# JihyongOh/DeMFI

Hardware: AMD Instinct MI355X
Metric: interpolated frames/sec @720p x8 MFI (N_tst=3) (higher is better)
Workload: dtype f16; 1 GPU; DeMFI-Net_rb N_tst=3, x8 MFI, 720x1280 (padded 736x1280), fp16, clip-parallel windows, random-init weights; uint8 frames host->HBM->host inside the timed region (PNG codec excluded), 8 distinct windows; graph=True, parallelism=clip1, n_ctx=7, n_trunk=3

## Files before the change

demfi_amd/_lib.py:

```python
import ctypes as C
import os

_HERE = os.path.dirname(os.path.abspath(__file__))
LIB_PATH = os.environ.get('DEMFI_HIP_LIB') or os.path.join(_HERE, 'csrc', 'libdemfi_hip.so')

F16, F32 = 0, 1
ABI_VERSION = 8
ACT_NONE, ACT_RELU, ACT_TANH, ACT_SIGMOID = 0, 1, 2, 3
MODE_STORE, MODE_MUL, MODE_GRU = 0, 1, 2
BT601, BT709 = 0, 1
SITING_420JPEG, SITING_420MPEG2 = 0, 1
YUV_LAYOUT = {'420': 0, '422': 1, '444': 2, 'mono': 3}
OWNERS = ('sep', 'wstream7', 'ws2', 'wstream3', 'c64', 'narrow_nhwc', 'narrow_thin', 'general')
OWNERS_COUT_PERM = frozenset(range(6))
MAX_PIECES, MAX_CHUNKS, MAX_SEGS, MAX_OCTS = 48, 40, 8, 32


class View(C.Structure):
    _fields_ = [('ptr', C.c_void_p), ('sx', C.c_int64), ('sy', C.c_int64), ('sc', C.c_int64), ('sb', C.c_int64),
                ('is_f32', C.c_int32), ('_pad', C.c_int32)]


class Piece(C.Structure):
    _fields_ = [('v', View), ('nch', C.c_int32), ('lds_ch', C.c_int32), ('up_shift', C.c_int32), ('fat', C.c_int32)]
# ... 176 lines not shown
                                   C.POINTER(C.c_int64)]),
    'demfi_png_info': (C.c_int, [C.c_void_p, C.c_int64, C.POINTER(C.c_int), C.POINTER(C.c_int)]),
    'demfi_png_decode': (C.c_int, [C.c_void_p, C.c_int64, C.c_void_p, C.c_int64, C.c_int, C.c_int]),
    'demfi_conv_build': (C.c_int, [C.c_int, C.c_int, C.c_int, C.c_int, C.c_int, C.c_void_p, C.c_void_p, C.c_int, C.c_int,
                                   C.c_int, C.c_int, C.POINTER(ConvSrc), C.c_int, C.POINTER(ConvDst), C.c_int, C.POINTER(Conv),
                                   C.c_void_p, C.POINTER(C.c_int64), C.c_void_p, C.POINTER(C.c_int32)]),
    'demfi_ctx_create': (C.c_int, [C.c_int, C.c_int, C.c_int, C.c_int, C.POINTER(HParams), C.c_int, C.c_int,
                                   C.POINTER(C.c_void_p)]),
    'demfi_ctx_destroy': (C.c_int, [C.c_void_p]),
    'demfi_gru_sep_create': (C.c_int, [C.c_int, C.c_int, C.c_int, C.c_int, C.POINTER(C.c_void_p)]),
    'demfi_fgac_create': (C.c_int, [C.c_int, C.c_int, C.c_int, C.c_int, C.POINTER(C.c_void_p)]),
    'demfi_operator_run': (C.c_int, [C.c_void_p, C.c_void_p]),
    'demfi_load_weight': (C.c_int, [C.c_void_p, C.c_char_p, C.c_void_p, C.POINTER(C.c_int64), C.c_int]),
    'demfi_ctx_workspace_bytes': (C.c_int64, [C.c_void_p]),
    'demfi_workspace_bytes': (C.c_int64, [C.c_int, C.c_int, C.c_int, C.c_int, C.c_int, C.c_int]),
    'demfi_ctx_bind': (C.c_int, [C.c_void_p, C.c_void_p, C.c_int64, C.c_int, C.c_void_p]),
    'demfi_ctx_weight_region': (C.c_int, [C.c_void_p, C.POINTER(C.c_int64), C.POINTER(C.c_int64)]),
    'demfi_ctx_buffer': (C.c_int, [C.c_void_p, C.c_int, C.c_int, C.c_char_p, C.POINTER(C.c_int64), C.POINTER(C.c_int32),
                                   C.POINTER(C.c_int32)]),
    'demfi_ingest_u8': (C.c_int, [C.c_void_p, C.c_int, C.c_void_p, C.c_int, C.c_int, C.c_void_p]),
    'demfi_ingest_u16': (C.c_int, [C.c_void_p, C.c_int, C.c_void_p, C.c_int, C.c_int, C.c_int, C.c_void_p]),
    'demfi_ingest_u16_rect': (C.c_int, [C.c_void_p, C.c_int, C.c_void_p, C.c_int, C.c_int, C.c_int, C.c_int, C.c_int, C.c_int, C.c_int,
                                        C.c_void_p]),
    'demfi_forward_trunk_body': (C.c_int, [C.c_void_p, C.c_int, C.c_void_p]),
    'demfi_forward_trunk': (C.c_int, [C.c_void_p, C.c_int, C.c_void_p, C.c_void_p]),
    'demfi_forward_t': (C.c_int, [C.c_void_p, C.c_int, C.c_int, C.c_int, C.c_void_p]),
    'demfi_forward_tb': (C.c_int, [C.c_void_p, C.c_int, C.c_int, C.c_void_p]),
    'demfi_forward_tb_final': (C.c_int, [C.c_void_p, C.c_int, C.c_int, C.c_void_p]),
    'demfi_ctx_num_ops': (C.c_int, [C.c_void_p, C.c_int, C.c_int, C.c_int, C.c_int]),
    'demfi_ctx_get_op': (C.c_int, [C.c_void_p, C.c_int, C.c_int, C.c_int, C.c_int, C.c_int, C.POINTER(Op)]),
    'demfi_ctx_num_convs': (C.c_int, [C.c_void_p]),
    'demfi_ctx_conv_desc': (C.POINTER(Conv), [C.c_void_p, C.c_int]),
    'demfi_conv_owner': (C.c_int, [C.POINTER(Conv)]),
    'demfi_run_op': (C.c_int, [C.c_void_p, C.POINTER(Op), C.c_void_p]),
    'demfi_graph_begin': (C.c_int, [C.c_void_p]),
    'demfi_graph_end': (C.c_int, [C.c_void_p, C.POINTER(C.c_void_p)]),
    'demfi_graph_launch': (C.c_int, [C.c_void_p, C.c_void_p]),
    'demfi_graph_destroy': (C.c_int, [C.c_void_p]),
}

EXPORTS = tuple(_SIGS)
_lib = None


class DemfiError(RuntimeError):
    pass


def load():
    global _lib
    if _lib is not None:
        return _lib
    if not os.path.exists(LIB_PATH):
        raise RuntimeError('demfi_amd: %s not found -- build it with demfi_amd/csrc/build.sh (or '
                           '__graft_entry__.build()); there is no CPU/PyTorch fallback for the forward path'
                           % LIB_PATH)
    lib = C.CDLL(LIB_PATH)
    for name, (res, args) in _SIGS.items():
        fn = getattr(lib, name)
        fn.restype = res
        fn.argtypes = args
    if lib.demfi_abi_version() != ABI_VERSION:
        raise RuntimeError('demfi_amd: ABI version mismatch')
    _lib = lib
    return lib

# ... 16 lines not shown
```

demfi_amd/csrc/conv.hip:

```cpp
#include "conv_common.h"

namespace {

static bool persist_out_eligible(const demfi_conv* h, bool allow_tanh = false);

bool persist_eligible(const demfi_conv* h)
{
    if (h->dtype != DEMFI_F16 || h->stride != 1 || h->kh != 3 || h->kw != 3 || h->pad_y != 1 || h->pad_x != 1) return false;
    if (h->n_chunks != 1 || h->n_pieces != 1 || h->chunks[0].nks != 4 || h->rec_bytes != 128) return false;
    const demfi_piece& p = h->pieces[0];
    if (!p.fat || p.nch != 64 || p.up_shift != 0 || !p.v.ptr || p.v.is_f32) return false;
    if (!persist_out_eligible(h, h->nco == 2)) return false;
    return demfi_c64_strides_ok(h);
}

static bool thin_out_eligible(const demfi_conv* h)
{
    if (h->nco != 1 || h->cout_pad != 32 || !h->zero_page || h->inH != h->H || h->inW != h->W || h->sub_seg[0] >= 0) return false;
    bool any = false;
    for (int g = 0; g < 4; ++g) {
        if (h->oct_n[g] == 0) continue;
        any = true;
        const demfi_seg& sg = h->segs[h->oct_seg[g]];
        if (sg.mode != DEMFI_MODE_STORE || sg.scale != 1 || sg.dy != 0 || sg.dx != 0) return false;
// ... 121 lines not shown
        if (!ok) return demfi_set_error(DEMFI_ERR_ARG, "demfi_conv2d: subtile %d is not eligible for the staged epilogue", sb);
    }
    hipStream_t st = (hipStream_t)stream;
    const int owner = demfi_conv_owner(h);
    if (h->pack.ptr != nullptr) {
        bool ok = owner == DEMFI_OWNER_NARROW_THIN && h->pack.sc == 1 && !h->pack.is_f32;
        for (int g = 0; g < 4; ++g) ok = ok && (h->pack_oct_ch[g] < 0 || (h->pack_oct_ch[g] % 4 == 0 && h->oct_n[g] > 0));
        if (!ok) return demfi_set_error(DEMFI_ERR_ARG, "demfi_conv2d: packed copy (demfi_conv.pack) on a layer that is not a thin-output fp16 narrow layer, or malformed");
    }
    if ((h->cout_perm != 0) != demfi_persist_eligible(h))
        return demfi_set_error(DEMFI_ERR_ARG, h->cout_perm ? "demfi_conv2d: descriptor packed for a persistent kernel (cout_perm) but not eligible for one (zero_page missing?)"
                                                           : "demfi_conv2d: persistent-kernel layer without cout_perm (build the descriptor with demfi_conv_build)");
    switch (owner) {
    case DEMFI_OWNER_SEP: return demfi_sep_launch(h, dev, st);
    case DEMFI_OWNER_WSTREAM7: return demfi_wstream_launch(h, dev, st);
    case DEMFI_OWNER_WS2: return demfi_ws2_launch(h, dev, st);
    case DEMFI_OWNER_WSTREAM3: return demfi_wstream3_launch(h, dev, st);
    case DEMFI_OWNER_C64: return demfi_c64_launch(h, dev, st);
    case DEMFI_OWNER_NARROW_NHWC: return demfi_narrow_launch(h, dev, st, false);
    case DEMFI_OWNER_NARROW_THIN: return demfi_narrow_launch(h, dev, st, true);
    default: return demfi_conv_general_launch(h, dev, st, (size_t)lds);
    }
}

#ifdef DEMFI_TRACE
extern "C" int demfi_trace_dump(unsigned long long* out, int64_t n)
{
    const int64_t have = TR_N;
    if (!out || n < have) return demfi_set_error(DEMFI_ERR_ARG, "demfi_trace_dump: need room for %lld entries", (long long)have);
    DEMFI_HIP_CHECK(hipDeviceSynchronize());
    for (int64_t i = 0; i < have; ++i) out[i] = 0;
    int st = demfi_c64_trace_collect(out);
    if (st >= 0) st = demfi_narrow_trace_collect(out);
    if (st >= 0) st = demfi_sep_trace_collect(out);
    if (st >= 0) st = demfi_wstream_trace_collect(out);
    return st < 0 ? st : (int)have;
}
#endif
```

demfi_amd/csrc/conv_kernels.h:

```cpp
#pragma once
#include <hip/hip_runtime.h>
#include "demfi_hip.h"

int demfi_conv_general_launch(const demfi_conv* h, const demfi_conv* dev, hipStream_t st, size_t lds);
int demfi_c64_launch(const demfi_conv* h, const demfi_conv* dev, hipStream_t st);
bool demfi_c64_strides_ok(const demfi_conv* h);
int demfi_narrow_launch(const demfi_conv* h, const demfi_conv* dev, hipStream_t st, bool thin);
bool demfi_sep_eligible(const demfi_conv* h);
int demfi_sep_launch(const demfi_conv* h, const demfi_conv* dev, hipStream_t st);
bool demfi_wstream_eligible(const demfi_conv* h, int ks = 7, int nch = 2);
int demfi_wstream_launch(const demfi_conv* h, const demfi_conv* dev, hipStream_t st);
int demfi_wstream3_launch(const demfi_conv* h, const demfi_conv* dev, hipStream_t st);
int demfi_c64_trace_collect(unsigned long long* acc);
int demfi_narrow_trace_collect(unsigned long long* acc);
int demfi_sep_trace_collect(unsigned long long* acc);
int demfi_wstream_trace_collect(unsigned long long* acc);
```

demfi_amd/csrc/conv_narrow.hip:

```cpp
#include "conv_common.h"

namespace {

template <int REC, int KS = 3> struct NarrowCfg {
    static constexpr int LW = TW + KS - 1, LH = TH + KS - 1, NP = LW * LH, PAD = KS / 2, NTAPS = KS * KS;
    static constexpr int NKS = REC / 32;
    static constexpr int SL = REC / 16;
    static constexpr int PPI = 1024 / REC;
    static constexpr int NI = (NP + PPI - 1) / PPI;
    static constexpr int TILE_BYTES = NI * 1024;
#ifndef DEMFI_N64_NBUF
#define DEMFI_N64_NBUF 3
#define DEMFI_N64_NDMA 4
#define DEMFI_N32_NDMA 2
#endif
    static constexpr int NBUF = REC == 128 ? 2 : (REC == 64 ? DEMFI_N64_NBUF : 4);
    static_assert(KS == 3 || (KS == 7 && REC == 32), "7x7: one 16-channel k-step per tap (49 KiB of resident weights)");
    static constexpr int NDMA = REC == 128 ? 4 : (REC == 64 ? DEMFI_N64_NDMA : (KS == 7 ? 2 : DEMFI_N32_NDMA));
    static_assert((NBUF - 1) * ((NI + NDMA - 1) / NDMA) <= 63, "a DMA wave's tiles in flight must be countable in vmcnt");
    static __device__ __forceinline__ int swz(int col) { return REC == 128 ? (col >> 1) & 7 : (REC == 64 ? (col >> 2) & 3 : (col >> 4) & 1); }
    static constexpr size_t lds_bytes(int nco) { return (size_t)NTAPS * NKS * nco * 1024 + (size_t)NBUF * TILE_BYTES + 1024; }
};

struct NarrowFrag { uint4 a[2], b0, b1; };

__device__ __forceinline__ void quad_transpose4(float (&a)[4], int lane)
{
    auto dpp = [](float v, auto CTRL) {
        return __builtin_bit_cast(float, __builtin_amdgcn_update_dpp(0, __builtin_bit_cast(int, v), decltype(CTRL)::value, 0xF, 0xF, false));
    };
    const bool b0 = lane & 1, b1 = lane & 2;
    float p[4], y[4], q[4];
#pragma unroll
    for (int j = 0; j < 4; ++j) p[j] = dpp(a[j], std::integral_constant<int, 0xB1>{});
    y[0] = b0 ? p[1] : a[0]; y[1] = b0 ? a[1] : p[0]; y[2] = b0 ? p[3] : a[2]; y[3] = b0 ? a[3] : p[2];
#pragma unroll
    for (int j = 0; j < 4; ++j) q[j] = dpp(y[j], std::integral_constant<int, 0x4E>{});
    a[0] = b1 ? q[2] : y[0]; a[1] = b1 ? q[3] : y[1]; a[2] = b1 ? y[2] : q[0]; a[3] = b1 ? y[3] : q[1];
}
#ifndef DEMFI_THIN_REGW_G128
#define DEMFI_THIN_REGW_G128 6
#endif
template <int NCO, int REC, int EPI, int KS = 3, int NDMA = NarrowCfg<REC, KS>::NDMA, int NOCT = 4, bool PACK = false, bool P7 = false>
__global__ __launch_bounds__(NT + 64 * NDMA, 1) void conv3x3_narrow_persist_kernel(const demfi_conv* __restrict__ d)
{
    static_assert(!P7 || (KS == 7 && NCO == 1 && REC == 32), "paired taps: the 7x7 / 16-channel / 32-cout instantiation");
    constexpr bool RES = EPI == 1, THIN = EPI == 2;
    constexpr bool REGW = THIN && KS == 3 && NCO == 1;
    constexpr int RG = (REGW && REC == 128 && NOCT == 1 && !PACK) ? DEMFI_THIN_REGW_G128 : 0;
    constexpr bool WLDS = RG < (REC / 32) * 3 || !REGW;
    static_assert(!PACK || THIN, "packed copy: thin epilogue only");
    static_assert(!THIN || NCO == 1, "thin epilogue: one 32-cout subtile");
    using Cfg = NarrowCfg<REC, KS>;
    constexpr int P_LW = Cfg::LW, P_NP = Cfg::NP, PAD = Cfg::PAD;
    constexpr int NKS = Cfg::NKS, SL = Cfg::SL, NI = Cfg::NI, NBUF = Cfg::NBUF, TILE_BYTES = Cfg::TILE_BYTES;
// ... 403 lines not shown
                    for (int p = 0; p < 2; ++p) quad_transpose4(vv[g][p], lane);
                }
#pragma unroll
                for (int g = 0; g < NOCT; ++g) {
#pragma unroll
                    for (int p = 0; p < 2; ++p) {
#pragma unroll
                        for (int j = 0; j < 4; ++j) vv[g][p][j] = vv[g][p][j] + tr[g][p][j];
                    }
                    apply_act_n<4>(vv[g][0], t_act[g]);
                    apply_act_n<4>(vv[g][1], t_act[g]);
                }
#pragma unroll
                for (int g = 0; g < NOCT; ++g) {
#pragma unroll
                    for (int p = 0; p < 2; ++p) {
                        const int oyv = oy0 + wave * 2 + p;
                        if (oyv < H && q4 < t_nq[g]) {
                            f4_t o;
#pragma unroll
                            for (int j = 0; j < 4; ++j) o[j] = vv[g][p][j];
                            *gp<f4_t>(t_dstq[g] + bimg * t_dsb[g] + (int64_t)oyv * t_dsy[g] + ox0 + (lx & ~3)) = o;
                        }
                    }
                }
                if constexpr (PACK) {
#pragma unroll
                    for (int g = 0; g < NOCT; ++g) {
                        if (pk_dst[g] == nullptr) continue;
#pragma unroll
                        for (int p = 0; p < 2; ++p) {
                            quad_transpose4(vv[g][p], lane);
                            const int oyv = oy0 + wave * 2 + p;
                            if (oyv < H) {
                                h4_t o;
#pragma unroll
                                for (int j = 0; j < 4; ++j) o[j] = j < t_nq[g] ? (half_t)vv[g][p][j] : (half_t)0.0f;
                                *gp<h4_t>(pk_dst[g] + bimg * pk_sb + (int64_t)oyv * pk_sy + (int64_t)(ox0 + lx) * pk_sx) = o;
                            }
                        }
                    }
                }
                TRACE_STAMP(wave, k, 3);
                continue;
            }
#pragma unroll
            for (int g = 0; g < NOCT; ++g) {
                if (t_on[g] == 0) continue;
                const f4_t bq = t_bias[g];
#pragma unroll
                for (int p = 0; p < 2; ++p) {
                    float v[4];
#pragma unroll
                    for (int j = 0; j < 4; ++j) v[j] = (acc[0][p][g * 4 + j] + bq[j]) + tr[g][p][j];
                    apply_act_n<4>(v, t_act[g]);
                    const int oy = oy0 + wave * 2 + p, oxx = ox0 + lx;
                    if (s_dst[g] != nullptr) {
                        if (hi == 0 && oy < s_h && oxx < s_w) {
                            unsigned char* bp = s_dst[g] + ((int64_t)oy * s_w + oxx) * 3;
#pragma unroll
                            for (int j = 0; j < 3; ++j) {
                                double q = ((double)v[j] + 1.0) / 2.0;
                                q = q < 0.0 ? 0.0 : (q > 1.0 ? 1.0 : q);
                                *gp<unsigned char>(bp + j) = (unsigned char)(q * 255.0);
                            }
                        }
                        continue;
                    }
                    if (oy < H && oxx < W) {
                        float* dp = t_dst[g] + bimg * t_dsb[g] + (int64_t)oy * t_dsy[g] + (int64_t)oxx * t_dsx[g];
#pragma unroll
                        for (int j = 0; j < 4; ++j)
                            if (j < t_nq[g]) *gp<float>(dp + j * t_dsc[g]) = v[j];
                        if (PACK && pk_dst[g] != nullptr) {
                            h4_t o;
#pragma unroll
                            for (int j = 0; j < 4; ++j) o[j] = j < t_nq[g] ? (half_t)v[j] : (half_t)0.0f;
                            *gp<h4_t>(pk_dst[g] + bimg * pk_sb + (int64_t)oy * pk_sy + (int64_t)oxx * pk_sx) = o;
                        }
                    }
                }
            }
            TRACE_STAMP(wave, k, 3);
            continue;
        }
        if constexpr (RES) {
#pragma unroll
            for (int s = 0; s < NCO; ++s) {
#pragma unroll
                for (int q = 0; q < 4; ++q) asm volatile("" : "+v"(rreg[s][q >> 1][q & 1]));
            }
        }
#pragma unroll
        for (int s = 0; s < NCO; ++s) {
#pragma unroll
            for (int m2 = 0; m2 < 2; ++m2) {
                const f4_t b0 = *(const f4_t*)(bias_lds + s * 32 + (2 * m2) * 8 + hi * 4);
                const f4_t b1 = *(const f4_t*)(bias_lds + s * 32 + (2 * m2 + 1) * 8 + hi * 4);
#pragma unroll
                for (int p = 0; p < 2; ++p) {
                    float v[8];
#pragma unroll
                    for (int j = 0; j < 4; ++j) {
                        v[j] = acc[s][p][(2 * m2) * 4 + j] + b0[j];
                        v[4 + j] = acc[s][p][(2 * m2 + 1) * 4 + j] + b1[j];
                    }
                    if constexpr (RES) {
                        const h8_t r = __builtin_bit_cast(h8_t, rreg[s][p][m2]);
#pragma unroll
                        for (int j = 0; j < 8; ++j) v[j] += (float)r[j];
                    }
#pragma unroll
// ... 42 lines not shown
            else if (noct == 3) hipLaunchKernelGGL((conv3x3_narrow_persist_kernel<1, REC, 2, KS, ND, 3>), dim3(grid), blk, lds, st, dev);
            else                hipLaunchKernelGGL((conv3x3_narrow_persist_kernel<1, REC, 2, KS>), dim3(grid), blk, lds, st, dev);
        } else
            return demfi_set_error(DEMFI_ERR_ARG, "demfi_conv2d: thin epilogue needs nco == 1");
    } else if (h->segs[h->sub_seg[0]].res.ptr != nullptr)
        hipLaunchKernelGGL((conv3x3_narrow_persist_kernel<NCO, REC, 1, KS>), dim3(grid), dim3(NT + 64 * NarrowCfg<REC, KS>::NDMA), lds, st, dev);
    else {
        if constexpr (KS == 7 && NCO == 1 && REC == 32) {
            const demfi_chunk& ch = h->chunks[0];
            if (ch.n_pieces == 2 && h->pieces[ch.first_piece].nch == 8 && h->pieces[ch.first_piece].v.ptr && h->pieces[ch.first_piece].lds_ch == 0 &&
                h->pieces[ch.first_piece + 1].v.ptr == nullptr) {
                constexpr int ND = 4;
                DEMFI_LDS_ATTR((conv3x3_narrow_persist_kernel<1, 32, 0, 7, ND, 4, false, true>));
                hipLaunchKernelGGL((conv3x3_narrow_persist_kernel<1, 32, 0, 7, ND, 4, false, true>), dim3(grid), dim3(NT + 64 * ND), lds, st, dev);
                DEMFI_HIP_CHECK(hipGetLastError());
                return DEMFI_OK;
            }
        }
        hipLaunchKernelGGL((conv3x3_narrow_persist_kernel<NCO, REC, 0, KS>), dim3(grid), dim3(NT + 64 * NarrowCfg<REC, KS>::NDMA), lds, st, dev);
    }
    DEMFI_HIP_CHECK(hipGetLastError());
    return DEMFI_OK;
}


}

int demfi_narrow_trace_collect(unsigned long long* acc) { return TRACE_DRAIN(acc, true); }

int demfi_narrow_launch(const demfi_conv* h, const demfi_conv* dev, hipStream_t st, bool thin)
{
    if (h->kh == 7) {
        if (!thin) return launch_narrow<1, 32, 7>(h, dev, st, false);
    } else
    switch (h->chunks[0].nks * 2 + h->nco) {
    case 1 * 2 + 1: return launch_narrow<1, 32>(h, dev, st, thin);
    case 1 * 2 + 2: return launch_narrow<2, 32>(h, dev, st, thin);
    case 2 * 2 + 1: return launch_narrow<1, 64>(h, dev, st, thin);
    case 2 * 2 + 2: return launch_narrow<2, 64>(h, dev, st, thin);
    case 4 * 2 + 1: return launch_narrow<1, 128>(h, dev, st, thin);
    case 4 * 2 + 2: return launch_narrow<2, 128>(h, dev, st, thin);
    }
    return demfi_set_error(DEMFI_ERR_ARG, "demfi_narrow_launch: not a narrow layer (kh=%d nks=%d nco=%d thin=%d)", h->kh, h->chunks[0].nks, h->nco, (int)thin);
}
```

include/demfi_hip.h:

```cpp
#ifndef DEMFI_HIP_H
#define DEMFI_HIP_H

#include <stdint.h>

#ifdef __cplusplus
extern "C" {
#endif

#define DEMFI_ABI_VERSION 8

enum demfi_dtype { DEMFI_F16 = 0, DEMFI_F32 = 1 };

enum demfi_status {
    DEMFI_OK = 0,
    DEMFI_ERR_ARG = -1,
    DEMFI_ERR_HIP = -2,
    DEMFI_ERR_NODEV = -3
};

enum demfi_yuv_matrix { DEMFI_BT601 = 0, DEMFI_BT709 = 1 };
enum demfi_chroma_siting { DEMFI_420JPEG = 0, DEMFI_420MPEG2 = 1 };
enum demfi_yuv_layout { DEMFI_YUV_420 = 0, DEMFI_YUV_422 = 1, DEMFI_YUV_444 = 2, DEMFI_YUV_MONO = 3 };

enum demfi_act { DEMFI_ACT_NONE = 0, DEMFI_ACT_RELU = 1, DEMFI_ACT_TANH = 2, DEMFI_ACT_SIGMOID = 3 };
// ... 320 lines not shown
    demfi_view a, b, o;
    const void* p[32];
    const void* t;
    char name[64];
    demfi_batch bt;
} demfi_op;

int     demfi_ctx_create(int H, int W, int max_updates, int dtype, const demfi_hparams* hp ,
                         int n_trunk, int n_ctx, demfi_ctx** out);
int     demfi_ctx_destroy(demfi_ctx* ctx);
int     demfi_load_weight(demfi_ctx* ctx, const char* name, const float* host, const int64_t* shape, int ndim);
int64_t demfi_ctx_workspace_bytes(const demfi_ctx* ctx);
int64_t demfi_workspace_bytes(int H, int W, int max_updates, int dtype, int n_trunk, int n_ctx);
int     demfi_ctx_bind(demfi_ctx* ctx, void* workspace, int64_t bytes, int on_host, void* stream);
int     demfi_ctx_weight_region(const demfi_ctx* ctx, int64_t* offset, int64_t* bytes);
int     demfi_ctx_buffer(const demfi_ctx* ctx, int trunk, int c, const char* name, int64_t* offset, int32_t* kind,
                         int32_t dims[4]);
int     demfi_ingest_u8(demfi_ctx* ctx, int trunk, const uint8_t* const* frames, int h, int w, void* stream);
int     demfi_ingest_u16(demfi_ctx* ctx, int trunk, const uint16_t* const* frames, int h, int w, int depth, void* stream);
int     demfi_ingest_u16_rect(demfi_ctx* ctx, int trunk, const uint16_t* const* frames, int fh, int fw, int y0, int x0, int h, int w,
                              int depth, void* stream);
int     demfi_forward_trunk_body(demfi_ctx* ctx, int trunk, void* stream);
int     demfi_forward_trunk(demfi_ctx* ctx, int trunk, const float* x, void* stream);
int     demfi_forward_t(demfi_ctx* ctx, int trunk, int c, int n_updates, void* stream);
int     demfi_forward_tb(demfi_ctx* ctx, int trunk, int n_updates, void* stream);
int     demfi_forward_tb_final(demfi_ctx* ctx, int trunk, int n_updates, void* stream);
int     demfi_ctx_num_ops(const demfi_ctx* ctx, int segment, int trunk, int c, int iter);
int     demfi_ctx_get_op(const demfi_ctx* ctx, int segment, int trunk, int c, int iter, int index, demfi_op* out);
int     demfi_ctx_num_convs(const demfi_ctx* ctx);
const demfi_conv* demfi_ctx_conv_desc(const demfi_ctx* ctx, int index);
enum demfi_owner { DEMFI_OWNER_SEP = 0, DEMFI_OWNER_WSTREAM7 = 1, DEMFI_OWNER_WS2 = 2, DEMFI_OWNER_WSTREAM3 = 3, DEMFI_OWNER_C64 = 4,
                   DEMFI_OWNER_NARROW_NHWC = 5, DEMFI_OWNER_NARROW_THIN = 6, DEMFI_OWNER_GENERAL = 7 };
int     demfi_conv_owner(const demfi_conv* desc);
int     demfi_run_op(demfi_ctx* ctx, const demfi_op* op, void* stream);

int demfi_gru_sep_create(int batch, int H, int W, int dtype, demfi_ctx** out);
int demfi_fgac_create(int batch, int H, int W, int dtype, demfi_ctx** out);
int demfi_operator_run(demfi_ctx* ctx, void* stream);

int demfi_graph_begin(void* stream);
int demfi_graph_end(void* stream, void** graph_exec_out);
int demfi_graph_launch(void* graph_exec, void* stream);
int demfi_graph_destroy(void* graph_exec);

#ifdef __cplusplus
}
#endif
#endif
```

Baseline: 103.4 frames/s.

## Add tap-expanded MFMA kernel for thin single-output 3x3 convolutions

Adds a new kernel for 3x3 convolutions with very few output channels. It spreads the 9 taps times couts across the MFMA output columns and then sums the taps through LDS, so the matrix units are not mostly idle on padded output channels. By default it is used only for layers with a single output channel; a runtime switch extends it to all eligible thin layers. The shared narrow config and pack/sink helpers move into a header. The trade-off is the extra LDS reduction, more barriers, and a separate code path to maintain.

After: 103.6 frames/s, median of 3. About the same (+0.2%).

```diff
diff --git a/demfi_amd/_lib.py b/demfi_amd/_lib.py
--- a/demfi_amd/_lib.py
+++ b/demfi_amd/_lib.py
@@ -232,6 +232,8 @@
     'demfi_ctx_num_convs': (C.c_int, [C.c_void_p]),
     'demfi_ctx_conv_desc': (C.POINTER(Conv), [C.c_void_p, C.c_int]),
     'demfi_conv_owner': (C.c_int, [C.POINTER(Conv)]),
+    'demfi_thin_path': (C.c_int, [C.POINTER(Conv)]),
+    'demfi_thin_tapx_all': (C.c_int, [C.c_int]),
     'demfi_run_op': (C.c_int, [C.c_void_p, C.POINTER(Op), C.c_void_p]),
     'demfi_graph_begin': (C.c_int, [C.c_void_p]),
     'demfi_graph_end': (C.c_int, [C.c_void_p, C.POINTER(C.c_void_p)]),
diff --git a/demfi_amd/csrc/conv.hip b/demfi_amd/csrc/conv.hip
--- a/demfi_amd/csrc/conv.hip
+++ b/demfi_amd/csrc/conv.hip
@@ -177,6 +177,7 @@
     for (int64_t i = 0; i < have; ++i) out[i] = 0;
     int st = demfi_c64_trace_collect(out);
     if (st >= 0) st = demfi_narrow_trace_collect(out);
+    if (st >= 0) st = demfi_thin_tapx_trace_collect(out);
     if (st >= 0) st = demfi_sep_trace_collect(out);
     if (st >= 0) st = demfi_wstream_trace_collect(out);
     return st < 0 ? st : (int)have;
diff --git a/demfi_amd/csrc/conv_kernels.h b/demfi_amd/csrc/conv_kernels.h
--- a/demfi_amd/csrc/conv_kernels.h
+++ b/demfi_amd/csrc/conv_kernels.h
@@ -6,6 +6,8 @@
 int demfi_c64_launch(const demfi_conv* h, const demfi_conv* dev, hipStream_t st);
 bool demfi_c64_strides_ok(const demfi_conv* h);
 int demfi_narrow_launch(const demfi_conv* h, const demfi_conv* dev, hipStream_t st, bool thin);
+bool demfi_thin_tapx_takes(const demfi_conv* h);
+int demfi_thin_tapx_launch(const demfi_conv* h, const demfi_conv* dev, hipStream_t st);
 bool demfi_sep_eligible(const demfi_conv* h);
 int demfi_sep_launch(const demfi_conv* h, const demfi_conv* dev, hipStream_t st);
 bool demfi_wstream_eligible(const demfi_conv* h, int ks = 7, int nch = 2);
@@ -13,5 +15,6 @@
 int demfi_wstream3_launch(const demfi_conv* h, const demfi_conv* dev, hipStream_t st);
 int demfi_c64_trace_collect(unsigned long long* acc);
 int demfi_narrow_trace_collect(unsigned long long* acc);
+int demfi_thin_tapx_trace_collect(unsigned long long* acc);
 int demfi_sep_trace_collect(unsigned long long* acc);
 int demfi_wstream_trace_collect(unsigned long long* acc);
diff --git a/demfi_amd/csrc/conv_narrow.h b/demfi_amd/csrc/conv_narrow.h
--- /dev/null
+++ b/demfi_amd/csrc/conv_narrow.h
@@ -0,0 +1,40 @@
+#pragma once
+#include "conv_common.h"
+
+namespace {
+
+template <int REC, int KS = 3> struct NarrowCfg {
+    static constexpr int LW = TW + KS - 1, LH = TH + KS - 1, NP = LW * LH, PAD = KS / 2, NTAPS = KS * KS;
+    static constexpr int NKS = REC / 32;
+    static constexpr int SL = REC / 16;
+    static constexpr int PPI = 1024 / REC;
+    static constexpr int NI = (NP + PPI - 1) / PPI;
+    static constexpr int TILE_BYTES = NI * 1024;
+#ifndef DEMFI_N64_NBUF
+#define DEMFI_N64_NBUF 3
+#define DEMFI_N64_NDMA 4
+#define DEMFI_N32_NDMA 2
+#endif
+    static constexpr int NBUF = REC == 128 ? 2 : (REC == 64 ? DEMFI_N64_NBUF : 4);
+    static_assert(KS == 3 || (KS == 7 && REC == 32), "7x7: one 16-channel k-step per tap (49 KiB of resident weights)");
+    static constexpr int NDMA = REC == 128 ? 4 : (REC == 64 ? DEMFI_N64_NDMA : (KS == 7 ? 2 : DEMFI_N32_NDMA));
+    static_assert((NBUF - 1) * ((NI + NDMA - 1) / NDMA) <= 63, "a DMA wave's tiles in flight must be countable in vmcnt");
+    static __device__ __forceinline__ int swz(int col) { return REC == 128 ? (col >> 1) & 7 : (REC == 64 ? (col >> 2) & 3 : (col >> 4) & 1); }
+    static constexpr size_t lds_bytes(int nco) { return (size_t)NTAPS * NKS * nco * 1024 + (size_t)NBUF * TILE_BYTES + 1024; }
+};
+
+__device__ __forceinline__ unsigned char thin_sink_u8(float v)
+{
+    double q = ((double)v + 1.0) / 2.0;
+    q = q < 0.0 ? 0.0 : (q > 1.0 ? 1.0 : q);
+    return (unsigned char)(q * 255.0);
+}
+__device__ __forceinline__ h4_t thin_pack4(const float (&v)[4], int nq)
+{
+    h4_t o;
+#pragma unroll
+    for (int j = 0; j < 4; ++j) o[j] = j < nq ? (half_t)v[j] : (half_t)0.0f;
+    return o;
+}
+
+}
diff --git a/demfi_amd/csrc/conv_narrow.hip b/demfi_amd/csrc/conv_narrow.hip
--- a/demfi_amd/csrc/conv_narrow.hip
+++ b/demfi_amd/csrc/conv_narrow.hip
@@ -1,26 +1,6 @@
-#include "conv_common.h"
+#include "conv_narrow.h"
 
 namespace {
-
-template <int REC, int KS = 3> struct NarrowCfg {
-    static constexpr int LW = TW + KS - 1, LH = TH + KS - 1, NP = LW * LH, PAD = KS / 2, NTAPS = KS * KS;
-    static constexpr int NKS = REC / 32;
-    static constexpr int SL = REC / 16;
-    static constexpr int PPI = 1024 / REC;
-    static constexpr int NI = (NP + PPI - 1) / PPI;
-    static constexpr int TILE_BYTES = NI * 1024;
-#ifndef DEMFI_N64_NBUF
-#define DEMFI_N64_NBUF 3
-#define DEMFI_N64_NDMA 4
-#define DEMFI_N32_NDMA 2
-#endif
-    static constexpr int NBUF = REC == 128 ? 2 : (REC == 64 ? DEMFI_N64_NBUF : 4);
-    static_assert(KS == 3 || (KS == 7 && REC == 32), "7x7: one 16-channel k-step per tap (49 KiB of resident weights)");
-    static constexpr int NDMA = REC == 128 ? 4 : (REC == 64 ? DEMFI_N64_NDMA : (KS == 7 ? 2 : DEMFI_N32_NDMA));
-    static_assert((NBUF - 1) * ((NI + NDMA - 1) / NDMA) <= 63, "a DMA wave's tiles in flight must be countable in vmcnt");
-    static __device__ __forceinline__ int swz(int col) { return REC == 128 ? (col >> 1) & 7 : (REC == 64 ? (col >> 2) & 3 : (col >> 4) & 1); }
-    static constexpr size_t lds_bytes(int nco) { return (size_t)NTAPS * NKS * nco * 1024 + (size_t)NBUF * TILE_BYTES + 1024; }
-};
 
 struct NarrowFrag { uint4 a[2], b0, b1; };
 
@@ -490,12 +470,7 @@
                         for (int p = 0; p < 2; ++p) {
                             quad_transpose4(vv[g][p], lane);
                             const int oyv = oy0 + wave * 2 + p;
-                            if (oyv < H) {
-                                h4_t o;
-#pragma unroll
-                                for (int j = 0; j < 4; ++j) o[j] = j < t_nq[g] ? (half_t)vv[g][p][j] : (half_t)0.0f;
-                                *gp<h4_t>(pk_dst[g] + bimg * pk_sb + (int64_t)oyv * pk_sy + (int64_t)(ox0 + lx) * pk_sx) = o;
-                            }
+                            if (oyv < H) *gp<h4_t>(pk_dst[g] + bimg * pk_sb + (int64_t)oyv * pk_sy + (int64_t)(ox0 + lx) * pk_sx) = thin_pack4(vv[g][p], t_nq[g]);
                         }
                     }
                 }
@@ -517,11 +492,7 @@
                         if (hi == 0 && oy < s_h && oxx < s_w) {
                             unsigned char* bp = s_dst[g] + ((int64_t)oy * s_w + oxx) * 3;
 #pragma unroll
-                            for (int j = 0; j < 3; ++j) {
-                                double q = ((double)v[j] + 1.0) / 2.0;
-                                q = q < 0.0 ? 0.0 : (q > 1.0 ? 1.0 : q);
-                                *gp<unsigned char>(bp + j) = (unsigned char)(q * 255.0);
-                            }
+                            for (int j = 0; j < 3; ++j) *gp<unsigned char>(bp + j) = thin_sink_u8(v[j]);
                         }
                         continue;
                     }
@@ -530,12 +501,8 @@
 #pragma unroll
                         for (int j = 0; j < 4; ++j)
                             if (j < t_nq[g]) *gp<float>(dp + j * t_dsc[g]) = v[j];
-                        if (PACK && pk_dst[g] != nullptr) {
-                            h4_t o;
-#pragma unroll
-                            for (int j = 0; j < 4; ++j) o[j] = j < t_nq[g] ? (half_t)v[j] : (half_t)0.0f;
-                            *gp<h4_t>(pk_dst[g] + bimg * pk_sb + (int64_t)oy * pk_sy + (int64_t)oxx * pk_sx) = o;
-                        }
+                        if (PACK && pk_dst[g] != nullptr)
+                            *gp<h4_t>(pk_dst[g] + bimg * pk_sb + (int64_t)oy * pk_sy + (int64_t)oxx * pk_sx) = thin_pack4(v, t_nq[g]);
                     }
                 }
             }
@@ -644,6 +611,8 @@
 {
     if (h->kh == 7) {
         if (!thin) return launch_narrow<1, 32, 7>(h, dev, st, false);
+    } else if (thin && demfi_thin_tapx_takes(h)) {
+        return demfi_thin_tapx_launch(h, dev, st);
     } else
     switch (h->chunks[0].nks * 2 + h->nco) {
     case 1 * 2 + 1: return launch_narrow<1, 32>(h, dev, st, thin);
@@ -655,3 +624,8 @@
     }
     return demfi_set_error(DEMFI_ERR_ARG, "demfi_narrow_launch: not a narrow layer (kh=%d nks=%d nco=%d thin=%d)", h->kh, h->chunks[0].nks, h->nco, (int)thin);
 }
+
+extern "C" int demfi_thin_path(const demfi_conv* h)
+{
+    return h && demfi_conv_owner(h) == DEMFI_OWNER_NARROW_THIN && demfi_thin_tapx_takes(h) ? 1 : 0;
+}
diff --git a/demfi_amd/csrc/conv_thin_tapx.hip b/demfi_amd/csrc/conv_thin_tapx.hip
--- /dev/null
+++ b/demfi_amd/csrc/conv_thin_tapx.hip
@@ -0,0 +1,430 @@
+#include "conv_narrow.h"
+
+namespace {
+
+constexpr int TX_MAXCO = 10;
+constexpr int TX_GROUPS = 11;
+constexpr int TX_GS = TX_GROUPS * 32;
+constexpr int TX_GBYTES = 32 * TX_GS * 4;
+constexpr int TX_PKG = 4;
+constexpr int TX_SCR = TX_PKG * 4 * NT * 4;
+constexpr int TX_TAB = 256;
+
+template <typename T> __device__ __forceinline__ T ldc(const void* p) { return *(const __attribute__((address_space(4))) T*)p; }
+
+struct TxPack { half_t* dst; int nq, sinkable, seg, pad; };
+static_assert(sizeof(TxPack) * TX_PKG + 4 <= TX_TAB, "tables");
+
+template <int REC> constexpr size_t tx_lds_bytes() { return (size_t)NarrowCfg<REC>::NBUF * NarrowCfg<REC>::TILE_BYTES + TX_GBYTES + TX_SCR + TX_TAB; }
+
+template <int REC, int NB>
+__global__ __launch_bounds__(NT + 64 * NarrowCfg<REC>::NDMA, 1) void conv3x3_thin_tapx_kernel(const demfi_conv* __restrict__ d)
+{
+    using Cfg = NarrowCfg<REC>;
+    constexpr int P_LW = Cfg::LW, P_NP = Cfg::NP, PAD = Cfg::PAD;
+    constexpr int NKS = Cfg::NKS, SL = Cfg::SL, NI = Cfg::NI, NBUF = Cfg::NBUF, TILE_BYTES = Cfg::TILE_BYTES, NDMA = Cfg::NDMA;
+    extern __shared__ __attribute__((aligned(16))) char smem[];
+    const int tid = threadIdx.x;
+    const int lane = tid & 63;
+    const int wave = __builtin_amdgcn_readfirstlane(tid >> 6);
+    const int H = d->H, W = d->W;
+    const int tiles_x = (W + TW - 1) / TW;
+    const int tiles_y = (H + TH - 1) / TH;
+    const int tiles_img = tiles_x * tiles_y;
+    const int total = tiles_img * d->batch;
+    char* const tbuf = smem;
+    float* const G = (float*)(smem + NBUF * TILE_BYTES);
+    float* const scr = (float*)(smem + NBUF * TILE_BYTES + TX_GBYTES);
+    TxPack* const ptab = (TxPack*)(smem + NBUF * TILE_BYTES + TX_GBYTES + TX_SCR);
+    int* const n_ptab = (int*)(ptab + TX_PKG);
+    int t_first, t_end, t_step;
+    XCD_TILE_STRIDE(total, t_first, t_end, t_step);
+    if (t_first >= t_end) return;
+    const int n_tiles = (t_end - t_first + t_step - 1) / t_step;
+    auto tile_coords = [&](int t, int& bimg, int& oy0, int& ox0) {
+        bimg = t / tiles_img;
+        const int rem = t - bimg * tiles_img;
+        const int ty = rem / tiles_x;
+        oy0 = ty * TH;
+        ox0 = (rem - ty * tiles_x) * TW;
+    };
+    const int co = d->oct_n[0] + d->oct_n[1] + d->oct_n[2] + d->oct_n[3];
+
+    float* c_dst[TX_MAXCO];
+    const float* c_res[TX_MAXCO];
+    int64_t c_dsb[TX_MAXCO], c_rsb[TX_MAXCO];
+    int c_sink[TX_MAXCO];
+    int c_pslot[TX_MAXCO];
+    float c_bias[TX_MAXCO];
+    {
+        int pk_base[4], gi = 0;
+#pragma unroll
+        for (int g = 0; g < 4; ++g) {
+            const bool on = d->pack.ptr != nullptr && d->pack_oct_ch[g] >= 0;
+            pk_base[g] = on ? gi * 4 : -1;
+            if (on) gi += (d->oct_n[g] + 3) >> 2;
+        }
+        static_for<0, TX_MAXCO>([&](auto C_) {
+            constexpr int ci = decltype(C_)::value;
+            int g = 0, j = ci;
+#pragma unroll
+            for (int q = 0; q < 3; ++q)
+                if (g == q && j >= d->oct_n[q]) { j -= d->oct_n[q]; g = q + 1; }
+            const bool live = ci < co;
+            const int sgi = d->oct_seg[g];
+            const demfi_seg& sg = d->segs[sgi];
+            const int c = d->oct_ch[g] + j;
+            c_dst[ci] = (float*)sg.dst.ptr + c * sg.dst.sc;
+            c_dsb[ci] = sg.dst.sb;
+            c_res[ci] = live && sg.res.ptr != nullptr ? (const float*)sg.res.ptr + c * sg.res.sc : nullptr;
+            c_rsb[ci] = sg.res.sb;
+            c_sink[ci] = d->oct_n[g] == 3 && d->oct_ch[g] == 0 ? (sgi << 4 | j) : -1;
+            c_pslot[ci] = pk_base[g] >= 0 ? pk_base[g] + j : -1;
+            c_bias[ci] = live ? *gcp<float>(d->bias + g * 8 + j) : 0.0f;
+        });
+    }
+    const int act = d->segs[d->oct_seg[0]].act;
+    if (tid == 64) {
+        int gi = 0;
+        if (d->pack.ptr != nullptr)
+            for (int g = 0; g < 4; ++g) {
+                if (d->pack_oct_ch[g] < 0) continue;
+                for (int h4 = 0; h4 * 4 < d->oct_n[g]; ++h4, ++gi) {
+                    TxPack p;
+                    p.dst = (half_t*)d->pack.ptr + d->pack_oct_ch[g] + 4 * h4;
+                    p.nq = min(4, d->oct_n[g] - 4 * h4);
+                    p.sinkable = (d->oct_n[g] == 3 && d->oct_ch[g] == 0) ? 1 : 0;
+                    p.seg = d->oct_seg[g]; p.pad = 0;
+                    ptab[gi] = p;
+                }
+            }
+        *n_ptab = gi;
+    }
+    for (int i = tid; i < TX_SCR / 4; i += blockDim.x) scr[i] = 0.0f;
+    __syncthreads();
+
+    if (wave >= 4) {
+        const int dw = wave - 4;
+        constexpr int NIW = NI / NDMA;
+        const demfi_chunk& ch = d->chunks[0];
+        const char* src[2] = {nullptr, nullptr};
+        int64_t psx[2] = {0, 0}, psy[2] = {0, 0}, psb[2] = {0, 0};
+        int pb0[2] = {0, 0}, pb1[2] = {0, 0};
+        int nreal = 0;
+        for (int k = 0; k < ch.n_pieces; ++k) {
+            const demfi_piece& pc = d->pieces[ch.first_piece + k];
+            if (pc.v.ptr == nullptr || nreal == 2) continue;
+            src[nreal] = (const char*)pc.v.ptr;
+            psx[nreal] = pc.v.sx * 2; psy[nreal] = pc.v.sy * 2; psb[nreal] = pc.v.sb * 2;
+            pb0[nreal] = pc.lds_ch * 2; pb1[nreal] = (pc.lds_ch + pc.nch) * 2;
+            ++nreal;
+        }
+        const char* const zeros = (const char*)d->zero_page;
+        int off[NI], meta[NI];
+        bool any_other = false;
+#pragma unroll
+        for (int i = 0; i < NI; ++i) {
+            const int px = i * Cfg::PPI + lane / SL;
+            const int pxc = min(px, P_NP - 1);
+            const int ly = pxc / P_LW;
+            const int lxx = pxc - ly * P_LW;
+            const int byte = (((lane & (SL - 1)) ^ Cfg::swz(lxx)) << 4);
+            int sel = 2;
+            if (byte >= pb0[0] && byte < pb1[0]) sel = 0;
+            else if (byte >= pb0[1] && byte < pb1[1]) sel = 1;
+            const int pi = sel == 1 ? 1 : 0;
+            off[i] = (int)(ly * psy[pi] + lxx * psx[pi]) + byte - pb0[pi];
+            meta[i] = px < P_NP ? (ly | (lxx << 8) | (sel << 16)) : (0xffff | (2 << 16));
+            any_other = any_other || sel != 0;
+        }
+        const bool simple = __builtin_amdgcn_readfirstlane(__ballot(any_other) == 0 ? 1 : 0) != 0;
+        auto issue_tile = [&](int k) {
+            int bimg, oy0, ox0;
+            tile_coords(t_first + k * t_step, bimg, oy0, ox0);
+            const char* base0 = src[0] + (int64_t)bimg * psb[0] + (int64_t)(oy0 - PAD) * psy[0] + (int64_t)(ox0 - PAD) * psx[0];
+            const char* base1 = src[1] + (int64_t)bimg * psb[1] + (int64_t)(oy0 - PAD) * psy[1] + (int64_t)(ox0 - PAD) * psx[1];
+            char* dst = tbuf + (k % NBUF) * TILE_BYTES;
+            const bool interior = oy0 >= PAD && oy0 + TH + PAD <= H && ox0 >= PAD && ox0 + TW + PAD <= W;
+            if (simple && interior) {
+#pragma unroll
+                for (int i = 0; i < NI; ++i) {
+                    if (NDMA > 1 && (i % NDMA) != dw) continue;
+                    __builtin_amdgcn_global_load_lds((const __attribute__((address_space(1))) void*)(base0 + off[i]),
+                                                     (__attribute__((address_space(3))) void*)(dst + i * 1024), 16, 0, 0);
+                }
+                return;
+            }
+#pragma unroll
+            for (int i = 0; i < NI; ++i) {
+                if (NDMA > 1 && (i % NDMA) != dw) continue;
+                int mt = meta[i];
+#if defined(__HIP_DEVICE_COMPILE__)
+                asm volatile("" : "+v"(mt));
+#endif
+                const int sel = mt >> 16;
+                const int iy = oy0 - PAD + (mt & 255), ix = ox0 - PAD + ((mt >> 8) & 255);
+                const bool ok = sel != 2 && (mt & 0xffff) != 0xffff && (interior || (iy >= 0 && iy < H && ix >= 0 && ix < W));
+                const char* g = ok ? (sel == 1 ? base1 : base0) + off[i] : zeros;
+                __builtin_amdgcn_global_load_lds((const __attribute__((address_space(1))) void*)g,
+                                                 (__attribute__((address_space(3))) void*)(dst + i * 1024), 16, 0, 0);
+            }
+        };
+        for (int k = 0; k < NBUF - 1 && k < n_tiles; ++k) issue_tile(k);
+        for (int k = 0; k < n_tiles; ++k) {
+            const int ahead = min(NBUF - 2, n_tiles - 1 - k);
+            if (ahead >= 2)      asm volatile("s_waitcnt vmcnt(%0)" ::"n"(2 * NIW <= 63 ? 2 * NIW : 0) : "memory");
+            else if (ahead == 1) asm volatile("s_waitcnt vmcnt(%0)" ::"n"(NIW <= 63 ? NIW : 0) : "memory");
+            else                 asm volatile("s_waitcnt vmcnt(0)" ::: "memory");
+            TRACE_STAMP(wave, k, 0);
+            asm volatile("s_barrier" ::: "memory");
+            TRACE_STAMP(wave, k, 1);
+            if (k + NBUF - 1 < n_tiles) issue_tile(k + NBUF - 1);
+            TRACE_STAMP(wave, k, 2);
+#pragma unroll
+            for (int i = 0; i < 2 * NB - 1; ++i) asm volatile("s_barrier" ::: "memory");
+        }
+        return;
+    }
+
+    const int hi = lane >> 5;
+    const int lx = lane & 31;
+    uint4 areg[NB][NKS];
+    {
+        const char* wg = (const char*)d->wpack;
+        static_for<0, NB>([&](auto B_) {
+            constexpr int b = decltype(B_)::value;
+            const int m = 32 * b + lx;
+            const int ci = m / 9, tap = m - ci * 9;
+            int prow = 0, jj = ci;
+            bool found = false;
+#pragma unroll
+            for (int g = 0; g < 4; ++g) {
+                const int n = d->oct_n[g];
+                if (!found && jj < n) { prow = g * 8 + jj; found = true; }
+                jj -= n;
+            }
+            static_for<0, NKS>([&](auto KS_) {
+                constexpr int ks = decltype(KS_)::value;
+                const char* p = found ? wg + (((tap * NKS + ks) * 64) + hi * 32 + prow) * 16 : (const char*)d->zero_page;
+                areg[b][ks] = ld_global16(p);
+            });
+        });
+    }
+#if defined(__HIP_DEVICE_COMPILE__)
+#pragma unroll
+    for (int b = 0; b < NB; ++b) {
+#pragma unroll
+        for (int ks = 0; ks < NKS; ++ks) asm volatile("" : "+v"(areg[b][ks].x), "+v"(areg[b][ks].y), "+v"(areg[b][ks].z), "+v"(areg[b][ks].w));
+    }
+#pragma unroll
+    for (int ci = 0; ci < TX_MAXCO; ++ci) asm volatile("" : "+v"(c_bias[ci]));
+#endif
+    int boff[3][NKS];
+#pragma unroll
+    for (int gi = 0; gi < 3; ++gi) {
+        const int q = min(32 * (wave + 4 * gi) + lx, P_NP - 1);
+        const int col = q % P_LW;
+#pragma unroll
+        for (int ks = 0; ks < NKS; ++ks) boff[gi][ks] = q * REC + (((ks * 2 + hi) ^ Cfg::swz(col)) << 4);
+    }
+    float* const gst = G + 4 * hi * TX_GS + 32 * wave + lx;
+    const int oyt = 2 * wave + hi;
+    const float* const gld = G + oyt * P_LW + lx;
+    float* const scrl = scr + tid;
+    const int npk = __builtin_amdgcn_readfirstlane(*n_ptab);
+    const int64_t pk_sx = d->pack.sx, pk_sy = d->pack.sy, pk_sb = d->pack.sb;
+    int64_t dsx = 0, dsy = 0, rsx = 0, rsy = 0;
+#pragma unroll
+    for (int g = 3; g >= 0; --g) {
+        if (d->oct_n[g] == 0) continue;
+        const demfi_seg& sg = d->segs[d->oct_seg[g]];
+        dsx = sg.dst.sx; dsy = sg.dst.sy;
+        if (sg.res.ptr != nullptr) { rsx = sg.res.sx; rsy = sg.res.sy; }
+    }
+    int slot = 0;
+    for (int k = 0; k < n_tiles; ++k) {
+        int bimg, oy0, ox0;
+        tile_coords(t_first + k * t_step, bimg, oy0, ox0);
+        const int oy = oy0 + oyt, ox = ox0 + lx;
+        const bool inb = oy < H && ox < W;
+        const int64_t dpix = (int64_t)oy * dsy + (int64_t)ox * dsx, rpix = (int64_t)oy * rsy + (int64_t)ox * rsx;
+        const char* sk = nullptr;
+        int s_h = 0, s_w = 0;
+        if (d->u8_sink != nullptr) {
+            const char* r = (const char*)d->u8_sink + (int64_t)bimg * DEMFI_U8_SINK_STRIDE;
+            if (ldc<int>(r + offsetof(demfi_u8_sink, iter)) == d->u8_iter) {
+                sk = r;
+                s_h = ldc<int>(r + offsetof(demfi_u8_sink, h));
+                s_w = ldc<int>(r + offsetof(demfi_u8_sink, w));
+            }
+        }
+        float rv[TX_MAXCO];
+        static_for<0, TX_MAXCO>([&](auto C_) {
+            constexpr int ci = decltype(C_)::value;
+            rv[ci] = 0.0f;
+            if (c_res[ci] != nullptr && inb) rv[ci] = *gcp<float>(c_res[ci] + bimg * c_rsb[ci] + rpix);
+        });
+        TRACE_STAMP(wave, k, 0);
+        asm volatile("s_waitcnt lgkmcnt(0)\n\ts_barrier" ::: "memory");
+        TRACE_STAMP(wave, k, 1);
+        f16x_t acc[3][NB];
+        const char* tb = tbuf + slot * TILE_BYTES;
+        slot = slot == NBUF - 1 ? 0 : slot + 1;
+        static_for<0, 3>([&](auto GI_) {
+            constexpr int gi = decltype(GI_)::value;
+            if (gi < 2 || wave < 3) {
+                uint4 bf[NKS];
+                static_for<0, NKS>([&](auto KS_) { bf[decltype(KS_)::value] = *(const uint4*)(tb + boff[gi][decltype(KS_)::value]); });
+                static_for<0, NKS>([&](auto KS_) {
+                    constexpr int ks = decltype(KS_)::value;
+                    static_for<0, NB>([&](auto B_) {
+                        constexpr int b = decltype(B_)::value;
+                        if constexpr (ks == 0) Mma<half_t>::init(acc[gi][b], areg[b][0], bf[0]);
+                        else Mma<half_t>::run(acc[gi][b], areg[b][ks], bf[ks]);
+                    });
+                });
+            }
+        });
+#if defined(DEMFI_TRACE) && defined(__HIP_DEVICE_COMPILE__)
+        static_for<0, 3 * NB>([&](auto I_) { asm volatile("" ::"v"(acc[decltype(I_)::value / NB][decltype(I_)::value % NB])); });
+        TRACE_STAMP(wave, k, 2);
+#endif
+#if defined(__HIP_DEVICE_COMPILE__)
+#pragma unroll
+        for (int ci = 0; ci < TX_MAXCO; ++ci) asm volatile("" : "+v"(rv[ci]));
+#endif
+        float out[TX_MAXCO];
+        static_for<0, NB>([&](auto B_) {
+            constexpr int b = decltype(B_)::value;
+            static_for<0, 3>([&](auto GI_) {
+                constexpr int gi = decltype(GI_)::value;
+                if (gi < 2 || wave < 3)
+                    static_for<0, 16>([&](auto R_) {
+                        constexpr int r = decltype(R_)::value;
+                        gst[(8 * (r >> 2) + (r & 3)) * TX_GS + 128 * gi] = acc[gi][b][r];
+                    });
+            });
+            asm volatile("s_waitcnt lgkmcnt(0)\n\ts_barrier" ::: "memory");
+            if constexpr (b == 0) TRACE_STAMP(wave, k, 4);
+            constexpr int NR = 9 * TX_MAXCO - 32 * b < 32 ? 9 * TX_MAXCO - 32 * b : 32;
+            float gv[NR];
+            static_for<0, NR>([&](auto M_) {
+                constexpr int ml = decltype(M_)::value, tap = (32 * b + ml) % 9;
+                gv[ml] = gld[ml * TX_GS + (tap / 3) * P_LW + (tap % 3)];
+            });
+            __builtin_amdgcn_sched_barrier(0);
+            static_for<0, NR>([&](auto M_) {
+                constexpr int ml = decltype(M_)::value, m = 32 * b + ml, ci = m / 9, tap = m % 9;
+                if constexpr (tap == 0) out[ci] = c_bias[ci] + gv[ml];
+                else out[ci] = out[ci] + gv[ml];
+                if constexpr (tap == 8) {
+                    if (ci < co) {
+                        float v[1] = {out[ci] + rv[ci]};
+                        apply_act_n<1>(v, act);
+                        unsigned char* fr = nullptr;
+                        if (sk != nullptr && c_sink[ci] >= 0) fr = ldc<unsigned char*>(sk + (c_sink[ci] >> 4) * 8);
+                        if (fr != nullptr) {
+                            if (oy < s_h && ox < s_w) *gp<unsigned char>(fr + ((int64_t)oy * s_w + ox) * 3 + (c_sink[ci] & 15)) = thin_sink_u8(v[0]);
+                        } else {
+                            if (inb) *gp<float>(c_dst[ci] + bimg * c_dsb[ci] + dpix) = v[0];
+                            if (c_pslot[ci] >= 0) scrl[c_pslot[ci] * NT] = v[0];
+                        }
+                    }
+                }
+            });
+            if constexpr (b + 1 < NB) asm volatile("s_waitcnt lgkmcnt(0)\n\ts_barrier" ::: "memory");
+        });
+        for (int gi = 0; gi < npk; ++gi) {
+            const TxPack& p = ptab[gi];
+            if (sk != nullptr && __builtin_amdgcn_readfirstlane(p.sinkable) && ldc<unsigned char*>(sk + __builtin_amdgcn_readfirstlane(p.seg) * 8) != nullptr) continue;
+            float v[4];
+#pragma unroll
+            for (int j = 0; j < 4; ++j) v[j] = scrl[(gi * 4 + j) * NT];
+            if (inb) *gp<h4_t>(p.dst + bimg * pk_sb + (int64_t)oy * pk_sy + (int64_t)ox * pk_sx) = thin_pack4(v, __builtin_amdgcn_readfirstlane(p.nq));
+        }
+        TRACE_STAMP(wave, k, 3);
+    }
+}
+
+template <int REC, int NB>
+int launch_tapx(const demfi_conv* h, const demfi_conv* dev, hipStream_t st)
+{
+    DEMFI_LDS_ATTR((conv3x3_thin_tapx_kernel<REC, NB>));
+    const int total = ((h->W + TW - 1) / TW) * ((h->H + TH - 1) / TH) * h->batch;
+    const int grid = total >= 256 ? 256 : total;
+    hipLaunchKernelGGL((conv3x3_thin_tapx_kernel<REC, NB>), dim3(grid), dim3(NT + 64 * NarrowCfg<REC>::NDMA), tx_lds_bytes<REC>(), st, dev);
+    DEMFI_HIP_CHECK(hipGetLastError());
+    return DEMFI_OK;
+}
+
+template <int REC>
+int launch_tapx_rec(const demfi_conv* h, const demfi_conv* dev, hipStream_t st, int nb)
+{
+    switch (nb) {
+    case 1: return launch_tapx<REC, 1>(h, dev, st);
+    case 2: return launch_tapx<REC, 2>(h, dev, st);
+    default: return launch_tapx<REC, 3>(h, dev, st);
+    }
+}
+
+int tx_couts(const demfi_conv* h) { return h->oct_n[0] + h->oct_n[1] + h->oct_n[2] + h->oct_n[3]; }
+
+}
+
+int demfi_thin_tapx_trace_collect(unsigned long long* acc) { return TRACE_DRAIN(acc, true); }
+
+static bool tx_shape_ok(const demfi_conv* h);
+
+static int g_tapx_all = 0;
+extern "C" int demfi_thin_tapx_all(int on)
+{
+    const int prev = g_tapx_all;
+    g_tapx_all = on ? 1 : 0;
+    return prev;
+}
+
+bool demfi_thin_tapx_takes(const demfi_conv* h)
+{
+    if (!tx_shape_ok(h)) return false;
+    return g_tapx_all != 0 || tx_couts(h) == 1;
+}
+
+static bool tx_shape_ok(const demfi_conv* h)
+{
+    if (h->kh != 3 || h->kw != 3 || h->nco != 1 || h->cout_pad != 32) return false;
+    const int nks = h->chunks[0].nks;
+    if (nks != 1 && nks != 2 && nks != 4) return false;
+    for (int g = 0; g < 4; ++g)
+        if (h->oct_n[g] < 0 || h->oct_n[g] > 8) return false;
+    const int co = tx_couts(h);
+    if (co < 1 || co > TX_MAXCO) return false;
+    const demfi_view *dv = nullptr, *rv = nullptr;
+    for (int g = 0; g < 4; ++g) {
+        if (h->oct_n[g] == 0) continue;
+        const demfi_seg& sg = h->segs[h->oct_seg[g]];
+        if (sg.act != h->segs[h->oct_seg[0]].act || h->oct_n[0] == 0) return false;
+        if (dv && (dv->sx != sg.dst.sx || dv->sy != sg.dst.sy)) return false;
+        dv = &sg.dst;
+        if (!sg.res.ptr) continue;
+        if (rv && (rv->sx != sg.res.sx || rv->sy != sg.res.sy)) return false;
+        rv = &sg.res;
+    }
+    if (h->pack.ptr != nullptr) {
+        int groups = 0;
+        for (int g = 0; g < 4; ++g)
+            if (h->pack_oct_ch[g] >= 0) groups += (h->oct_n[g] + 3) / 4;
+        if (groups > TX_PKG) return false;
+    }
+    return true;
+}
+
+int demfi_thin_tapx_launch(const demfi_conv* h, const demfi_conv* dev, hipStream_t st)
+{
+    const int nb = (9 * tx_couts(h) + 31) / 32;
+    switch (h->chunks[0].nks) {
+    case 1: return launch_tapx_rec<32>(h, dev, st, nb);
+    case 2: return launch_tapx_rec<64>(h, dev, st, nb);
+    case 4: return launch_tapx_rec<128>(h, dev, st, nb);
+    }
+    return demfi_set_error(DEMFI_ERR_ARG, "demfi_thin_tapx_launch: nks=%d", h->chunks[0].nks);
+}
diff --git a/include/demfi_hip.h b/include/demfi_hip.h
--- a/include/demfi_hip.h
+++ b/include/demfi_hip.h
@@ -376,6 +376,8 @@
 enum demfi_owner { DEMFI_OWNER_SEP = 0, DEMFI_OWNER_WSTREAM7 = 1, DEMFI_OWNER_WS2 = 2, DEMFI_OWNER_WSTREAM3 = 3, DEMFI_OWNER_C64 = 4,
                    DEMFI_OWNER_NARROW_NHWC = 5, DEMFI_OWNER_NARROW_THIN = 6, DEMFI_OWNER_GENERAL = 7 };
 int     demfi_conv_owner(const demfi_conv* desc);
+int     demfi_thin_path(const demfi_conv* desc);
+int     demfi_thin_tapx_all(int on);
 int     demfi_run_op(demfi_ctx* ctx, const demfi_op* op, void* stream);
 
 int demfi_gru_sep_create(int batch, int H, int W, int dtype, demfi_ctx** out);
```
